# ChuckDanz/DCLIP

Measured on AMD Instinct MI355X. Metric: distill-step images/sec at ViT-B/32 bs=256, higher is better.
Workload: dtype f32

## Files before the change

### dclip_amd/_lib.py

```python
from __future__ import annotations

import ctypes as C
import os

_HERE = os.path.dirname(os.path.abspath(__file__))
LIB_PATH = os.environ.get("DCLIP_LIB_PATH") or os.path.join(_HERE, "libdclip_hip.so")

P = C.c_void_p
I = C.c_int
F = C.c_float
Z = C.c_size_t
L = C.c_int64

SIGNATURES = {
    "dclip_abi_version": (I, []),
    "dclip_last_error": (C.c_char_p, []),
    "dclip_last_launch": (C.c_char_p, []),
    "dclip_first_launch": (C.c_char_p, []),
    "dclip_gemm_f32_workspace": (Z, [I, I, I, I, I]),
    "dclip_gemm_f32_plan": (I, [I, I, I, I, I, C.POINTER(C.c_int)]),
    "dclip_gemm_f32": (I, [P, P, P, P, P, P, I, I, I, I, I, I, I, I, F, I, P, Z, P]),
    "dclip_colsum_f32_workspace": (Z, [I, I]),
    "dclip_colsum_f32": (I, [P, P, I, I, I, I, P, Z, P]),
    "dclip_layernorm_fwd": (I, [P, P, P, P, P, P, I, I, F, P]),
# ... 103 lines not shown
    "dclip_split_f32_f16x3_dev": (I, [P, P, I, I, I, I, P, I, P]),
    "dclip_layernorm_fwd_f16x3_dev": (I, [P, P, P, P, P, P, P, I, I, F, P, P]),
    "dclip_gemm_f16_scaled_dev": (I, [P, P, P, P, P, I, I, I, I, I, I, I, I, P, P]),
    "dclip_gemm_f16_scaled_split_dev": (I, [P, P, P, P, P, P, I, I, I, I, I, I, I, P, P, P]),
    "dclip_split16_record_bytes": (I, []),
    "dclip_split16_plan_floats": (I, []),
    "dclip_split16_tile_rows": (I, []),
    "dclip_split16_stats": (I, [P, I, I, P, P]),
    "dclip_split16_plan": (I, [P, P, I, I, P]),
    "dclip_split16_weights": (I, [P, I, I, P, P]),
    "dclip_split_f32_f16x3_rows": (I, [P, P, P, I, I, I, P]),
    "dclip_split16_weights_t": (I, [P, I, I, P, P, P]),
    "dclip_gemm_f16_scaled_rows_dev": (I, [P, P, P, P, I, I, I, I, I, I, I, P, P, P]),
    "dclip_split_f32_f16x3_rows_colstats_workspace": (Z, [I, I]),
    "dclip_split_f32_f16x3_rows_colstats": (I, [P, P, P, P, P, P, P, I, I, I, P, Z, P]),
    "dclip_split_f32_f16x3_rows_cols_stats": (I, [P, P, P, P, P, P, P, P, P, I, I, I, I, P]),
    "dclip_gemm_f16_scaled_rows_stats_plan": (I, [I, I, I]),
    "dclip_gemm_f16_scaled_rows_stats_dev": (I, [P, P, P, P, I, I, I, I, I, I, I, P, P, P, P, P]),
    "dclip_attention_bwd_stats_plan": (I, [I, I, I]),
    "dclip_attention_bwd_stats": (I, [P, P, P, P, P, P, P, I, I, I, I, P]),
    "dclip_layernorm_bwd_stats_plan": (I, [I, I]),
    "dclip_layernorm_bwd_stats": (I, [P, P, P, P, P, P, P, P, P, P, P, I, I, I, P, Z, P]),
    "dclip_gemm_f16x3_plan": (I, [I, I, I]),
    "dclip_gemm_f16x3_scaled": (I, [P, P, P, P, P, I, I, I, I, I, I, I, I, I, I, I, I, F, P]),
    "dclip_gemm_f16x3_scaled_split": (I, [P, P, P, P, I, I, I, I, I, I, I, I, I, I, I, F, F, P]),
    "dclip_gemm_f16x3_scaled_dev": (I, [P, P, P, P, P, I, I, I, I, I, I, I, I, I, I, I, I, P, P]),
    "dclip_gemm_f16x3_scaled_split_dev": (I, [P, P, P, P, P, P, I, I, I, I, I, I, I, I, I, I, I, P, P, P]),
    "dclip_gemm_f16x3_scaled_rows_dev": (I, [P, P, P, P, I, I, I, I, I, I, I, I, I, I, I, P, P, P]),
    "dclip_gemm_f16x3_scaled_rows_stats_plan": (I, [I, I, I]),
    "dclip_gemm_f16x3_scaled_rows_stats_dev": (I, [P, P, P, P, I, I, I, I, I, I, I, I, I, I, I, P, P, P, P, P]),
    "dclip_gemm_f16x3_wgrad_tokmajor_plan": (I, [I, I, I]),
    "dclip_gemm_f16x3_wgrad_tokmajor_workspace": (Z, [I, I, I]),
    "dclip_gemm_f16x3_wgrad_tokmajor": (I, [P, P, P, I, I, I, I, I, I, I, I, I, I, P, P, I, P, Z, P]),
    "dclip_gemm_f16_wgrad_tokmajor_seg3_plan": (I, [I, I, I]),
    "dclip_gemm_f16_wgrad_tokmajor_seg3": (I, [P, P, P, I, I, I, I, I, I, I, I, I, I, I, I, P, P, I, P, Z, P]),
    "dclip_gemm_f16_ex": (I, [P, P, P, P, P, P, I, I, I, I, I, I, I, I, P]),
    "dclip_gemm_f16_wgrad_tokmajor_plan": (I, [I, I, I]),
    "dclip_gemm_f16_wgrad_tokmajor": (I, [P, P, P, I, I, I, I, I, I, I, P, Z, P]),
    "dclip_gemm_f16_splitk_plan": (I, [I, I, I]),
    "dclip_gemm_f16_splitk_workspace": (Z, [I, I, I]),
    "dclip_gemm_f16_splitk": (I, [P, P, P, I, I, I, I, I, I, I, P, Z, P]),
    "dclip_cast_f32_f16_ieee": (I, [P, P, I, I, I, I, P]),
    "dclip_layernorm_fwd_f16_stats": (I, [P, P, P, P, P, P, I, I, F, P]),
    "dclip_layernorm_bwd_ex_f16": (I, [P, P, P, P, P, P, P, P, P, P, P, I, I, I, P, Z, P]),
    "dclip_transpose_to_f16": (I, [P, I, P, P, I, I, I, I, I, P]),
    "dclip_rowsum_f16": (I, [P, P, I, I, I, P]),
# ... 40 lines not shown
```

### dclip_amd/csrc/gemm_bf16.hip

```cpp
#include "common.h"
#include <stdlib.h>
#include <type_traits>

namespace {

typedef unsigned short u16x4 __attribute__((ext_vector_type(4)));
typedef unsigned int u32x4 __attribute__((ext_vector_type(4)));
typedef unsigned int u32x2 __attribute__((ext_vector_type(2)));

constexpr int BKH = 64;

struct GemmBf16Params {
  const __bf16* A;
  const __bf16* W;
  void* C;
  const float* bias;
  const float* residual;
  int M, N, K;
  int lda, ldw, ldc;
  int epilogue;
  int out_bf16;
  int tiles_m, tiles_n;
  unsigned short* aux;
  int k_per_split;
// ... 273 lines not shown
__device__ __forceinline__ void dma16(__amdgpu_buffer_rsrc_t rsrc, __bf16* lds_dst, int voff, int soff) {
  __builtin_amdgcn_raw_ptr_buffer_load_lds(rsrc, (__attribute__((address_space(3))) void*)lds_dst, 16, voff, soff, 0, 0);
}

template <class T, int BM>
int launch_reg(const GemmBf16Params& p, size_t lds, hipStream_t st) {
  if constexpr (std::is_same<T, F16T>::value) {
    if (p.row_alpha) {
      hipLaunchKernelGGL((gemm_bf16_kernel<T, BM, BM, true>), dim3(p.tiles_m * p.tiles_n), dim3(256), lds, st, p);
      return DCLIP_OK;
    }
  }
  hipLaunchKernelGGL((gemm_bf16_kernel<T, BM, BM>), dim3(p.tiles_m * p.tiles_n), dim3(256), lds, st, p);
  return DCLIP_OK;
}

#define PP_BARRIER()                      \
  do {                                    \
    __builtin_amdgcn_sched_barrier(0);    \
    __builtin_amdgcn_s_barrier();         \
    __builtin_amdgcn_sched_barrier(0);    \
  } while (0)

template <class T, int KIND, bool OUT16, bool DEV = false, bool ROWS = false, bool STATS = false>
__device__ __forceinline__ void pp_epilogue(const GemmBf16Params& p, const f32x4 (&acc)[8][4], float* ct, int m0, int n0,
                                            int tid, int wr, int wc, int quad, int l15) {
  constexpr int BN = 256;
  const int lc = (tid & 63) * 4, col = n0 + lc, lr0 = tid >> 6;
  const bool colok = col < p.N;
  const int colc = colok ? col : 0;
  f32x4 bias4 = {0.f, 0.f, 0.f, 0.f};
  if (p.epilogue & DCLIP_EPI_BIAS) bias4 = *reinterpret_cast<const f32x4*>(p.bias + colc);
  const float alpha_d = DEV ? *p.alpha_p : 0.f;
  static_assert(!STATS || ROWS, "the statistics form is the row-scaled one");
  unsigned smx[STATS ? 4 : 1];
  float ssm[STATS ? 4 : 1];
  if constexpr (STATS) {
#pragma unroll
    for (int e = 0; e < 4; ++e) smx[e] = 0u, ssm[e] = 0.f;
  }
#pragma unroll
  for (int hm = 0; hm < 2; ++hm) {
    const int rbase = m0 + hm * 128 + lr0;
    f32x4 side[KIND == 3 || (ROWS && KIND == 2) ? 16 : 1];
    u16x4 side16[KIND == 2 && !ROWS ? 16 : 1];
    if (ROWS && KIND == 2) {
#pragma unroll
      for (int q = 0; q < 16; ++q)
        side[q] = *reinterpret_cast<const f32x4*>(p.aux32 + (size_t)min(rbase + 8 * q, p.M - 1) * p.ldc + colc);
    }
    if (KIND == 3) {
#pragma unroll
      for (int q = 0; q < 16; ++q)
        side[q] = *reinterpret_cast<const f32x4*>(p.residual + (size_t)min(rbase + 8 * q, p.M - 1) * p.ldc + colc);
    }
    if (KIND == 2 && !ROWS) {
#pragma unroll
      for (int q = 0; q < 16; ++q)
        side16[q] = *reinterpret_cast<const u16x4*>(p.aux + (size_t)min(rbase + 8 * q, p.M - 1) * p.ldc + colc);
    }
    if (wr == hm) {
#pragma unroll
      for (int i = 0; i < 8; ++i)
#pragma unroll
        for (int j = 0; j < 4; ++j)
          *reinterpret_cast<f32x4*>(ct + (16 * i + l15) * BN + (((16 * wc + 4 * j + quad) ^ (l15 & 7)) << 2)) = acc[i][j];
    }
    asm volatile("s_waitcnt lgkmcnt(0)" ::: "memory");
    PP_BARRIER();
#pragma unroll
    for (int q = 0; q < 16; ++q) {
      const int row = rbase + 8 * q;
      f32x4 v = *reinterpret_cast<const f32x4*>(ct + (lr0 + 8 * q) * BN + (((tid & 63) ^ ((lr0 + 8 * q) & 7)) << 2));
      if (!ROWS) v = v * (DEV ? alpha_d : p.alpha) + bias4;
      const size_t off = (size_t)row * p.ldc + col;
      const bool ok = row < p.M && colok;
      if (ROWS) {
        if (KIND == 2) {
#pragma unroll
          for (int e = 0; e < 4; ++e) v[e] *= quick_gelu_grad_f(side[q][e]);
        }
        if (ok) *reinterpret_cast<f32x4*>(reinterpret_cast<float*>(p.C) + off) = v;
        if constexpr (STATS) if (ok) {
#pragma unroll
          for (int e = 0; e < 4; ++e) {
            const float ve = v[e];
            const unsigned u = __builtin_bit_cast(unsigned, ve) & 0x7fffffffu;
            smx[e] = smx[e] > u ? smx[e] : u;
            ssm[e] += ve;
          }
        }
        continue;
      }
      if (KIND == 1) {
        if (DEV && !OUT16 && p.h32 && ok) *reinterpret_cast<f32x4*>(p.h32 + (size_t)row * p.N + col) = v;
        if (p.aux) {
          u16x4 h = {T::bits(v[0]), T::bits(v[1]), T::bits(v[2]), T::bits(v[3])};
          if (ok) *reinterpret_cast<u16x4*>(p.aux + off) = h;
#pragma unroll
          for (int e = 0; e < 4; ++e) v[e] = T::to_f32(h[e]);
        }
#pragma unroll
        for (int e = 0; e < 4; ++e) v[e] = quick_gelu_f(v[e]);
      }
      if (KIND == 2) {
#pragma unroll
        for (int e = 0; e < 4; ++e) v[e] *= quick_gelu_grad_f(T::to_f32(side16[q][e]));
      }
      if (KIND == 3) v += side[q];
      if (!ok) continue;
      if ((KIND == 0 || KIND == 1) && !OUT16 && p.out_scale != 0.f) {
        if (DEV && p.g32) *reinterpret_cast<f32x4*>(p.g32 + (size_t)row * p.N + col) = v;
        store_split4(reinterpret_cast<unsigned short*>(p.C) + off, p.N, v, DEV ? *p.out_scale_p : p.out_scale);
        continue;
      }
      if (OUT16) {
        u16x4 o = {T::bits(v[0]), T::bits(v[1]), T::bits(v[2]), T::bits(v[3])};
        *reinterpret_cast<u16x4*>(reinterpret_cast<unsigned short*>(p.C) + off) = o;
      } else {
        *reinterpret_cast<f32x4*>(reinterpret_cast<float*>(p.C) + off) = v;
      }
    }
    if (hm == 0) {
      asm volatile("s_waitcnt lgkmcnt(0)" ::: "memory");
      PP_BARRIER();
      PP_STAMP(3);
    }
  }
  PP_STAMP(8);
  if constexpr (STATS) {
    asm volatile("s_waitcnt lgkmcnt(0)" ::: "memory");
    PP_BARRIER();
    unsigned* cu = reinterpret_cast<unsigned*>(ct);
    float* cs = ct + 8 * BN;
// ... 61 lines not shown
    if (row >= p.M || col >= p.N) continue;
    const size_t off = (size_t)row * p.ldc + col;
    const bool full = col + 8 <= p.N;
    typedef unsigned short u16x8 __attribute__((ext_vector_type(8)));
    u16x8 o = {lo[0], lo[1], lo[2], lo[3], hi[0], hi[1], hi[2], hi[3]};
    if (SAVE) {
      if (full) *reinterpret_cast<u16x8*>(p.aux + off) = o;
      else *reinterpret_cast<u16x4*>(p.aux + off) = lo;
#pragma unroll
      for (int e = 0; e < 8; ++e) o[e] = T::bits(quick_gelu_f(T::to_f32(o[e])));
    }
    unsigned short* c = reinterpret_cast<unsigned short*>(p.C) + off;
    if (full) *reinterpret_cast<u16x8*>(c) = o;
    else *reinterpret_cast<u16x4*>(c) = u16x4{o[0], o[1], o[2], o[3]};
  }
  PP_STAMP(8);
#ifdef DCLIP_GEMM_STAMPS
  asm volatile("s_waitcnt vmcnt(0)" ::: "memory");
#endif
  PP_STAMP(4);
  PP_STAMP_RT(6);
}

template <class T, bool TOK, bool DEV = false, bool ROWS = false, bool SEG = false, bool STATS = false, bool FUSED = false>
__global__ void __launch_bounds__(512) gemm_bf16_pp_kernel(GemmBf16Params p) {
  static_assert(!SEG || (TOK && !DEV && !ROWS), "the segmented form is token-major, split-K, fp32 slabs");
  static_assert(!FUSED || !SEG, "the fused form does all three products in one work item");
  constexpr int KT = FUSED ? BKH / 2 : BKH;
  static_assert(!STATS || (ROWS && !TOK), "the statistics form is the row-scaled dgrad");
  typedef typename T::x8 V8;
  constexpr int BM = 256, BN = 256, ROW = BKH;
  constexpr int BUF = (BM + BN) * ROW;
  __shared__ __attribute__((aligned(16))) unsigned char lds_raw[2 * BUF * 2];
  __bf16* lds = reinterpret_cast<__bf16*>(lds_raw);

  PP_STAMP(0);
  PP_STAMP_RT(5);
  PP_STAMP_V(7, (unsigned long long)__builtin_amdgcn_s_getreg((4) | (0 << 6) | (31 << 11)) |
                    ((unsigned long long)__builtin_amdgcn_s_getreg((20) | (0 << 6) | (3 << 11)) << 32));
  const int tid = threadIdx.x, lane = tid & 63;
  const int wave = __builtin_amdgcn_readfirstlane(tid >> 6);
  const int wr = wave >> 2, wc = wave & 3;
  const int l15 = lane & 15, quad = lane >> 4;

  constexpr int GROUP_M = 8;
  const int nwg = p.tiles_m * p.tiles_n;
  const int swz = xcd_remap16(blockIdx.x, nwg);
  const int per_group = GROUP_M * p.tiles_n;
  const int first_m = (swz / per_group) * GROUP_M;
  const int gsize = min(GROUP_M, p.tiles_m - first_m);
  const int tile_m = first_m + (swz % per_group) % gsize, tile_n = (swz % per_group) / gsize;
  const int m0 = tile_m * BM, n0 = tile_n * BN;
  int ksplit = blockIdx.y, a_col0 = 0, w_col0 = 0;
  if constexpr (SEG) {
    const int seg = (int)blockIdx.y / p.seg_splits;
    ksplit = (int)blockIdx.y - seg * p.seg_splits;
// ... 11 lines not shown
         w_bytes = TOK ? ((size_t)(p.K - kbeg - 1) * p.ldw + w_rows) * 2 : ((size_t)(w_rows - 1) * p.ldw + (p.K - kbeg)) * 2;
  if constexpr (FUSED) {
    a_bytes += (size_t)max(p.a_seg[0], p.a_seg[1]) * 2;
    w_bytes += (size_t)max(p.w_seg[0], p.w_seg[1]) * 2;
  }
  const __amdgpu_buffer_rsrc_t a_rsrc =
      __builtin_amdgcn_make_buffer_rsrc(const_cast<__bf16*>(a_org), 0, (int)min(a_bytes, (size_t)0x7fffffff), 0x00020000);
  const __amdgpu_buffer_rsrc_t w_rsrc =
      __builtin_amdgcn_make_buffer_rsrc(const_cast<__bf16*>(w_org), 0, (int)min(w_bytes, (size_t)0x7fffffff), 0x00020000);
  const int a_kstep = TOK ? KT * p.lda * 2 : KT * 2, w_kstep = TOK ? KT * p.ldw * 2 : KT * 2;
  int a_voff[2][2], w_voff[2][2];
#pragma unroll
  for (int h = 0; h < 2; ++h)
#pragma unroll
    for (int x = 0; x < 2; ++x) {
      if constexpr (FUSED) {
        if (TOK) {
          const int k = 4 * (wave + 8 * x) + (lane >> 4), tok = k & 31;
          const int lg = (lane & 15) ^ (((k & 3) << 2) | (((k >> 3) & 1) << 1));
          const int ma = 128 * (lg >> 3) + 64 * h + 8 * (lg & 7), nb = 64 * (lg >> 2) + 32 * h + 8 * (lg & 3);
          a_voff[h][x] = ma < a_rows ? (tok * p.lda + p.a_seg[x] + ma) * 2 : 0x7fffffff;
          w_voff[h][x] = nb < w_rows ? (tok * p.ldw + p.w_seg[x] + nb) * 2 : 0x7fffffff;
        } else {
          const int ra = 128 * x + 64 * h + 8 * wave + (lane >> 3), ga = (lane & 7) ^ ((ra >> 1) & 7);
          a_voff[h][x] = ra < a_rows ? (ra * p.lda + (ga < 4 ? p.a_seg[0] : p.a_seg[1]) + (ga & 3) * 8) * 2 : 0x7fffffff;
          const int rb = 64 * (2 * x + (wave >> 2)) + 32 * h + 8 * (wave & 3) + (lane >> 3), gb = (lane & 7) ^ ((rb >> 1) & 7);
          w_voff[h][x] = rb < w_rows ? (rb * p.ldw + (gb < 4 ? p.w_seg[0] : p.w_seg[1]) + (gb & 3) * 8) * 2 : 0x7fffffff;
        }
      } else if (TOK) {
        const int k = 4 * (wave + 8 * x) + (lane >> 4);
        const int lg = (lane & 15) ^ (((k & 3) << 2) | (((k >> 3) & 1) << 1));
        const int ma = 128 * (lg >> 3) + 64 * h + 8 * (lg & 7), nb = 64 * (lg >> 2) + 32 * h + 8 * (lg & 3);
        a_voff[h][x] = ma < a_rows ? (k * p.lda + ma) * 2 : 0x7fffffff;
        w_voff[h][x] = nb < w_rows ? (k * p.ldw + nb) * 2 : 0x7fffffff;
      } else {
        const int ra = 128 * x + 64 * h + 8 * wave + (lane >> 3), ga = (lane & 7) ^ ((ra >> 1) & 7);
        a_voff[h][x] = ra < a_rows ? (ra * p.lda + ga * 8) * 2 : 0x7fffffff;
        const int rb = 64 * (2 * x + (wave >> 2)) + 32 * h + 8 * (wave & 3) + (lane >> 3), gb = (lane & 7) ^ ((rb >> 1) & 7);
        w_voff[h][x] = rb < w_rows ? (rb * p.ldw + gb * 8) * 2 : 0x7fffffff;
      }
    }
  constexpr int HALF = 64 * 128;
#define PP_ISSUE_A(h, buf, kt)                                                                                          \
  do {                                                                                                                  \
    if (TOK) {                                                                                                          \
      dma16(a_rsrc, lds + (buf) * BUF + (h) * HALF + wave * 512, a_voff[h][0], (kt) * a_kstep);                         \
      dma16(a_rsrc, lds + (buf) * BUF + (h) * HALF + (wave + 8) * 512, a_voff[h][1], (kt) * a_kstep);                   \
    } else {                                                                                                            \
      dma16(a_rsrc, lds + (buf) * BUF + (64 * (h) + 8 * wave) * ROW, a_voff[h][0], (kt) * a_kstep);                     \
      dma16(a_rsrc, lds + (buf) * BUF + (128 + 64 * (h) + 8 * wave) * ROW, a_voff[h][1], (kt) * a_kstep);               \
    }                                                                                                                   \
  } while (0)
#define PP_ISSUE_B(h, buf, kt)                                                                                          \
  do {                                                                                                                  \
    if (TOK) {                                                                                                          \
      dma16(w_rsrc, lds + (buf) * BUF + (2 + (h)) * HALF + wave * 512, w_voff[h][0], (kt) * w_kstep);                   \
      dma16(w_rsrc, lds + (buf) * BUF + (2 + (h)) * HALF + (wave + 8) * 512, w_voff[h][1], (kt) * w_kstep);             \
    } else {                                                                                                            \
      dma16(w_rsrc, lds + (buf) * BUF + (BM + 64 * (wave >> 2) + 32 * (h) + 8 * (wave & 3)) * ROW, w_voff[h][0],        \
            (kt) * w_kstep);                                                                                            \
      dma16(w_rsrc, lds + (buf) * BUF + (BM + 128 + 64 * (wave >> 2) + 32 * (h) + 8 * (wave & 3)) * ROW, w_voff[h][1],  \
            (kt) * w_kstep);                                                                                            \
    }                                                                                                                   \
  } while (0)

  const int sw = l15 >> 1;
  const __bf16* pa0 = lds + (128 * wr + l15) * ROW + (((0 + quad) ^ sw) << 3);
  const __bf16* pa1 = lds + (128 * wr + l15) * ROW + (((4 + quad) ^ sw) << 3);
  const __bf16* pb0 = lds + (BM + 64 * wc + l15) * ROW + (((0 + quad) ^ sw) << 3);
  const __bf16* pb1 = lds + (BM + 64 * wc + l15) * ROW + (((4 + quad) ^ sw) << 3);
  const unsigned char* lds8 = lds_raw;
  const int tq = l15 >> 2, swzl = (tq << 2) | ((quad & 1) << 1);
  const int trow = (8 * quad + tq) * 256 + 8 * (l15 & 1);
  int ta[4], tb[2];
#pragma unroll
  for (int i = 0; i < 4; ++i) ta[i] = trow + (((8 * wr + 2 * i + ((l15 & 3) >> 1)) ^ swzl) << 4);
#pragma unroll
  for (int j = 0; j < 2; ++j) tb[j] = trow + (((4 * wc + 2 * j + ((l15 & 3) >> 1)) ^ swzl) << 4);
  auto tr8 = [&](int byte_off) {
    typedef short s16x4_t __attribute__((ext_vector_type(4)));
    typedef short s16x8_t __attribute__((ext_vector_type(8)));
    const s16x4_t lo = __builtin_amdgcn_ds_read_tr16_b64_v4i16((__attribute__((address_space(3))) s16x4_t*)(lds8 + byte_off));
    const s16x4_t hi = __builtin_amdgcn_ds_read_tr16_b64_v4i16((__attribute__((address_space(3))) s16x4_t*)(lds8 + byte_off + 1024));
    return __builtin_bit_cast(V8, s16x8_t{lo[0], lo[1], lo[2], lo[3], hi[0], hi[1], hi[2], hi[3]});
  };

  f32x4 acc[8][4];
#pragma unroll
  for (int i = 0; i < 8; ++i)
#pragma unroll
    for (int j = 0; j < 4; ++j) acc[i][j] = f32x4{0.f, 0.f, 0.f, 0.f};
  V8 fa[4][2], fb0[2][2], fb1[2][2];

#define PP_READ_A(qm, off)                                                                          \
  _Pragma("unroll") for (int i = 0; i < 4; ++i) {                                                   \
    if (TOK) {                                                                                      \
      fa[i][0] = tr8((off) * 2 + (qm) * (HALF * 2) + ta[i]);                                        \
      fa[i][1] = tr8((off) * 2 + (qm) * (HALF * 2) + ta[i] + 32 * 256);                             \
    } else {                                                                                        \
      fa[i][0] = *reinterpret_cast<const V8*>(pa0 + (off) + (64 * (qm) + 16 * i) * ROW);        \
      fa[i][1] = *reinterpret_cast<const V8*>(pa1 + (off) + (64 * (qm) + 16 * i) * ROW);        \
    }                                                                                               \
  }
#define PP_READ_B(fb, qn, off)                                                                      \
  _Pragma("unroll") for (int j = 0; j < 2; ++j) {                                                   \
    if (TOK) {                                                                                      \
      fb[j][0] = tr8((off) * 2 + (2 + (qn)) * (HALF * 2) + tb[j]);                                  \
      fb[j][1] = tr8((off) * 2 + (2 + (qn)) * (HALF * 2) + tb[j] + 32 * 256);                       \
    } else {                                                                                        \
      fb[j][0] = *reinterpret_cast<const V8*>(pb0 + (off) + (32 * (qn) + 16 * j) * ROW);        \
      fb[j][1] = *reinterpret_cast<const V8*>(pb1 + (off) + (32 * (qn) + 16 * j) * ROW);        \
    }                                                                                               \
  }
#define PP_MFMA(qm, qn, fb)                                                                                         \
  do {                                                                                                              \
    __builtin_amdgcn_s_setprio(1);                                                                                  \
    _Pragma("unroll") for (int s = 0; s < (FUSED ? 3 : 2); ++s)                                                     \
    _Pragma("unroll") for (int i = 0; i < 4; ++i)                                                                   \
    _Pragma("unroll") for (int j = 0; j < 2; ++j)                                                                   \
      acc[4 * (qm) + i][2 * (qn) + j] =                                                                             \
          T::mfma16(fb[j][FUSED ? s >> 1 : s], fa[i][FUSED ? s & 1 : s], acc[4 * (qm) + i][2 * (qn) + j]);          \
    __builtin_amdgcn_s_setprio(0);                                                                                  \
  } while (0)

  PP_ISSUE_A(0, 0, 0);
  PP_ISSUE_B(0, 0, 0);
  PP_ISSUE_B(1, 0, 0);
  PP_ISSUE_A(1, 0, 0);
  if (nk > 1) {
    PP_ISSUE_B(0, 1, 1);
    PP_ISSUE_A(0, 1, 1);
    PP_ISSUE_B(1, 1, 1);
    asm volatile("s_waitcnt vmcnt(6)" ::: "memory");
  } else {
    asm volatile("s_waitcnt vmcnt(0)" ::: "memory");
  }
  PP_BARRIER();
  PP_STAMP(1);
  if (wr == 1) PP_BARRIER();

  for (int kt = 0; kt < nk; ++kt) {
    const int cur = kt & 1, off = cur * BUF;
    const bool n1 = kt + 1 < nk, n2 = kt + 2 < nk;
    PP_READ_B(fb0, 0, off);
    __builtin_amdgcn_sched_barrier(0);
    PP_READ_A(0, off);
    __builtin_amdgcn_sched_barrier(0);
    if (n1) PP_ISSUE_A(1, cur ^ 1, kt + 1);
    if (!TOK) asm volatile("s_waitcnt lgkmcnt(8)" ::: "memory");
    PP_BARRIER();
    asm volatile("s_waitcnt lgkmcnt(0)" ::: "memory");
    __builtin_amdgcn_sched_barrier(0);
    PP_MFMA(0, 0, fb0);
    PP_BARRIER();
    PP_READ_B(fb1, 1, off);
    __builtin_amdgcn_sched_barrier(0);
    if (!TOK && n2) PP_ISSUE_B(0, cur, kt + 2);
    PP_BARRIER();
    asm volatile("s_waitcnt lgkmcnt(0)" ::: "memory");
    __builtin_amdgcn_sched_barrier(0);
    PP_MFMA(0, 1, fb1);
    PP_BARRIER();
    PP_READ_A(1, off);
    __builtin_amdgcn_sched_barrier(0);
    if (n2) PP_ISSUE_A(0, cur, kt + 2);
    PP_BARRIER();
    asm volatile("s_waitcnt lgkmcnt(0)" ::: "memory");
    __builtin_amdgcn_sched_barrier(0);
    PP_MFMA(1, 1, fb1);
    PP_BARRIER();
    if (n2) {
      if (TOK) PP_ISSUE_B(0, cur, kt + 2);
      PP_ISSUE_B(1, cur, kt + 2);
      asm volatile("s_waitcnt vmcnt(6)" ::: "memory");
    } else {
      asm volatile("s_waitcnt vmcnt(0)" ::: "memory");
    }
    PP_BARRIER();
    PP_MFMA(1, 0, fb0);
    PP_BARRIER();
  }
  if (wr == 0) PP_BARRIER();
  PP_STAMP(2);
#undef PP_ISSUE_A
#undef PP_ISSUE_B
#undef PP_READ_A
#undef PP_READ_B
#undef PP_MFMA

  const int kind = (p.epilogue & DCLIP_EPI_RESIDUAL) ? 3 : (p.epilogue & DCLIP_EPI_DGELU) ? 2 : (p.epilogue & DCLIP_EPI_GELU) ? 1 : 0;
  float* ct = reinterpret_cast<float*>(lds_raw);
  if (ROWS) {
    const float alpha_r = *p.alpha_p;
    float ra[8];
#pragma unroll
    for (int i = 0; i < 8; ++i) ra[i] = p.row_alpha[min(m0 + 128 * wr + 16 * i + l15, p.M - 1)];
#pragma unroll
    for (int i = 0; i < 8; ++i)
#pragma unroll
      for (int j = 0; j < 4; ++j) acc[i][j] = (acc[i][j] * alpha_r) * ra[i];
    if (kind == 2) pp_epilogue<T, 2, false, true, true, STATS>(p, acc, ct, m0, n0, tid, wr, wc, quad, l15);
    else pp_epilogue<T, 0, false, true, true, STATS>(p, acc, ct, m0, n0, tid, wr, wc, quad, l15);
    return;
  }
  if (!DEV && p.slab) {
    GemmBf16Params ps = p;
    ps.C = p.slab + (size_t)blockIdx.y * p.M * p.N;
    ps.ldc = p.N;
    ps.epilogue = 0;
    ps.alpha = 1.f;
    ps.out_scale = 0.f;
    pp_epilogue<T, 0, false, false>(ps, acc, ct, m0, n0, tid, wr, wc, quad, l15);
    return;
  }
  if (p.out_bf16) {
    unsigned short* ct16 = reinterpret_cast<unsigned short*>(lds_raw);
    if (kind == 0) pp_epilogue_b16<T, false, false, DEV>(p, acc, ct16, m0, n0, tid, wr, wc, quad, l15);
    else if (kind == 1 && p.aux) pp_epilogue_b16<T, true, true, DEV>(p, acc, ct16, m0, n0, tid, wr, wc, quad, l15);
    else if (kind == 1) pp_epilogue_b16<T, true, false, DEV>(p, acc, ct16, m0, n0, tid, wr, wc, quad, l15);
    else pp_epilogue<T, 2, true, DEV>(p, acc, ct, m0, n0, tid, wr, wc, quad, l15);
  } else {
    if (kind == 0) pp_epilogue<T, 0, false, DEV>(p, acc, ct, m0, n0, tid, wr, wc, quad, l15);
    else if (kind == 1) pp_epilogue<T, 1, false, DEV>(p, acc, ct, m0, n0, tid, wr, wc, quad, l15);
    else if (kind == 2) pp_epilogue<T, 2, false, DEV>(p, acc, ct, m0, n0, tid, wr, wc, quad, l15);
    else pp_epilogue<T, 3, false, DEV>(p, acc, ct, m0, n0, tid, wr, wc, quad, l15);
  }
}
#undef PP_BARRIER

#define PP_BARRIER()                      \
  do {                                    \
    __builtin_amdgcn_sched_barrier(0);    \
    __builtin_amdgcn_s_barrier();         \
    __builtin_amdgcn_sched_barrier(0);    \
  } while (0)

template <class T>
__global__ void __launch_bounds__(512) gemm_bf16_ppp_kernel(GemmBf16Params p) {
// ... 577 lines not shown
DCLIP_API int dclip_gemm_f16_scaled_rows_stats_dev(const void* A, const void* W, float* C, const float* aux32, int M, int N, int K,
                                                   int lda, int ldw, int ldc, int epilogue, const float* alpha, const float* row_alpha,
                                                   void* pmax, float* psum, void* stream) {
  DCLIP_REQUIRE(alpha && row_alpha && ((uintptr_t)alpha | (uintptr_t)row_alpha) % 4 == 0,
                "gemm_f16_scaled_rows_stats_dev: alpha / row_alpha must be device pointers");
  DCLIP_REQUIRE(pmax && psum && ((uintptr_t)pmax | (uintptr_t)psum) % 4 == 0, "gemm_f16_scaled_rows_stats_dev: pmax / psum");
  DCLIP_REQUIRE(epilogue == 0 || epilogue == DCLIP_EPI_DGELU, "gemm_f16_scaled_rows_stats_dev: the epilogue is none or DGELU");
  DCLIP_REQUIRE(!(epilogue & DCLIP_EPI_DGELU) || (aux32 && (uintptr_t)aux32 % 16 == 0),
                "gemm_f16_scaled_rows_stats_dev: DGELU needs a 16-byte aligned fp32 aux32");
  DCLIP_REQUIRE(dclip_gemm_f16_scaled_rows_stats_plan(M, N, K) > 0,
                "gemm_f16_scaled_rows_stats_dev: M=%d N=%d K=%d takes a register-staged kernel, which has no statistics form", M, N, K);
  DevScales dev{alpha, nullptr, nullptr, nullptr};
  dev.row_alpha = row_alpha;
  dev.aux32 = (epilogue & DCLIP_EPI_DGELU) ? aux32 : nullptr;
  dev.pmax = (unsigned*)pmax;
  dev.psum = psum;
  return gemm16<F16T>("gemm_f16_scaled_rows_dev.stats", A, W, C, nullptr, nullptr, nullptr, M, N, K, lda, ldw, ldc, epilogue, 0, stream,
                      1.f, 0.f, &dev);
}

namespace {
struct Segs { int a_hi, a_lo, w_hi, w_lo; };

int gemm16x3(const char* name, const void* A, const void* W, void* C, const float* bias, const float* residual, int M, int N, int K,
             int lda, int ldw, int ldc, Segs sg, int epilogue, int out_f16, void* stream, float alpha, float out_scale,
             const DevScales* dev) {
  DCLIP_REQUIRE(A && W && C, "%s: null operand", name);
  DCLIP_REQUIRE(M > 0 && N > 0 && K > 0 && K % 32 == 0, "%s: bad shape M=%d N=%d K=%d (K: the logical length, a multiple of 32)", name,
                M, N, K);
  DCLIP_REQUIRE(lda % 8 == 0 && ldw % 8 == 0 && lda > 0 && ldw > 0, "%s: lda/ldw must be multiples of 8", name);
  DCLIP_REQUIRE(sg.a_hi >= 0 && sg.a_lo >= 0 && sg.w_hi >= 0 && sg.w_lo >= 0 && (sg.a_hi | sg.a_lo | sg.w_hi | sg.w_lo) % 8 == 0,
                "%s: segment offsets must be non-negative multiples of 8", name);
  DCLIP_REQUIRE((long)sg.a_hi + K <= lda && (long)sg.a_lo + K <= lda && (long)sg.w_hi + K <= ldw && (long)sg.w_lo + K <= ldw,
                "%s: a segment (offset + K) must lie within the leading dimension", name);
  DCLIP_REQUIRE(N % 4 == 0 && ldc % 4 == 0 && ldc >= N, "%s: N / ldc must be multiples of 4", name);
  DCLIP_REQUIRE(((uintptr_t)A | (uintptr_t)W | (uintptr_t)C) % 16 == 0, "%s: operands must be 16-byte aligned", name);
  DCLIP_REQUIRE(!(epilogue & ~(DCLIP_EPI_BIAS | DCLIP_EPI_GELU | DCLIP_EPI_DGELU | DCLIP_EPI_RESIDUAL)),
                "%s: unsupported epilogue bits", name);
  DCLIP_REQUIRE(out_scale == 0.f || (!out_f16 && !(epilogue & (DCLIP_EPI_RESIDUAL | DCLIP_EPI_DGELU)) && (long)ldc >= 3L * N),
                "%s: a split output takes BIAS | GELU only and ldc >= 3 N", name);
  DCLIP_REQUIRE(!(epilogue & DCLIP_EPI_DGELU) || (dev && dev->aux32 && !(epilogue & DCLIP_EPI_GELU)), "%s: DGELU needs aux32", name);
  DCLIP_REQUIRE(!(epilogue & DCLIP_EPI_BIAS) || bias, "%s: BIAS without bias", name);
  DCLIP_REQUIRE(!(epilogue & DCLIP_EPI_RESIDUAL) || (residual && !out_f16), "%s: RESIDUAL needs an fp32 output", name);
  DCLIP_REQUIRE(256L * lda * 2 < 0x7fffffffL && 256L * ldw * 2 < 0x7fffffffL, "%s: leading dimension too large", name);
  GemmBf16Params p{(const __bf16*)A, (const __bf16*)W, C, bias, residual, M, N, K, lda, ldw, ldc, epilogue, out_f16, cdiv(M, 256),
                   cdiv(N, 256), nullptr, 0, nullptr, alpha, out_scale};
  set_dev(p, dev);
  p.a_seg[0] = sg.a_hi, p.a_seg[1] = sg.a_lo, p.w_seg[0] = sg.w_hi, p.w_seg[1] = sg.w_lo;
  const dim3 grid(p.tiles_m * p.tiles_n), block(512);
  hipStream_t st = (hipStream_t)stream;
  if (p.row_alpha && p.pmax)
    hipLaunchKernelGGL((gemm_bf16_pp_kernel<F16T, false, true, true, false, true, true>), grid, block, 0, st, p);
  else if (p.row_alpha)
    hipLaunchKernelGGL((gemm_bf16_pp_kernel<F16T, false, true, true, false, false, true>), grid, block, 0, st, p);
  else if (p.alpha_p)
    hipLaunchKernelGGL((gemm_bf16_pp_kernel<F16T, false, true, false, false, false, true>), grid, block, 0, st, p);
  else
    hipLaunchKernelGGL((gemm_bf16_pp_kernel<F16T, false, false, false, false, false, true>), grid, block, 0, st, p);
  DCLIP_CHECK_LAUNCH_V(name, ".pp3");
  return DCLIP_OK;
}
}

DCLIP_API int dclip_gemm_f16x3_plan(int M, int N, int K) {
  if (M <= 0 || N <= 0 || K <= 0 || K % 32 != 0 || !takes_pp(M, N, 3 * K)) return 0;
  const int tiles_min = getenv("DCLIP_F16X3_MIN") ? atoi(getenv("DCLIP_F16X3_MIN")) : 128;
  return (long)cdiv(M, 256) * cdiv(N, 256) >= tiles_min ? 1 : 0;
}

DCLIP_API int dclip_gemm_f16x3_scaled(const void* A, const void* W, void* C, const float* bias, const float* residual, int M, int N,
                                      int K, int lda, int ldw, int ldc, int a_hi, int a_lo, int w_hi, int w_lo, int epilogue,
                                      int out_f16, float alpha, void* stream) {
  DCLIP_REQUIRE(!(epilogue & DCLIP_EPI_DGELU), "gemm_f16x3_scaled: DGELU is a training epilogue");
  DCLIP_REQUIRE(alpha == alpha && alpha - alpha == 0.f, "gemm_f16x3_scaled: alpha must be finite");
  return gemm16x3("gemm_f16x3_scaled", A, W, C, bias, residual, M, N, K, lda, ldw, ldc, Segs{a_hi, a_lo, w_hi, w_lo}, epilogue, out_f16,
                  stream, alpha, 0.f, nullptr);
}

DCLIP_API int dclip_gemm_f16x3_scaled_split(const void* A, const void* W, void* C, const float* bias, int M, int N, int K, int lda,
                                            int ldw, int ldc, int a_hi, int a_lo, int w_hi, int w_lo, int epilogue, float alpha,
                                            float out_scale, void* stream) {
  DCLIP_REQUIRE(alpha == alpha && alpha - alpha == 0.f, "gemm_f16x3_scaled_split: alpha must be finite");
  DCLIP_REQUIRE(out_scale > 0.f && out_scale - out_scale == 0.f && (__builtin_bit_cast(unsigned int, out_scale) & 0x007fffffu) == 0,
                "gemm_f16x3_scaled_split: out_scale must be a power of two");
  DCLIP_REQUIRE(ldc % 8 == 0, "gemm_f16x3_scaled_split: ldc must be a multiple of 8");
  return gemm16x3("gemm_f16x3_scaled_split", A, W, C, bias, nullptr, M, N, K, lda, ldw, ldc, Segs{a_hi, a_lo, w_hi, w_lo}, epilogue, 0,
                  stream, alpha, out_scale, nullptr);
}

DCLIP_API int dclip_gemm_f16x3_scaled_dev(const void* A, const void* W, void* C, const float* bias, const float* residual, int M,
// ... 385 lines not shown
```

### dclip_amd/ops.py

```python
from __future__ import annotations

from typing import Optional

import torch

from . import _lib

A_KMAJOR, B_KMAJOR = 1, 2
EPI_BIAS, EPI_GELU, EPI_DGELU, EPI_RESIDUAL, EPI_ACCUM, EPI_A_ROWSUM = 1, 2, 4, 8, 16, 32
LAYOUT_NT = A_KMAJOR | B_KMAJOR
LAYOUT_NN = A_KMAJOR
LAYOUT_TN = 0


def _stream():
    return torch.cuda.current_stream().cuda_stream


def _f32(t: torch.Tensor, name: str) -> torch.Tensor:
    if not (t.is_cuda and t.dtype == torch.float32 and t.is_contiguous()):
        raise ValueError(f"{name}: expected a contiguous float32 CUDA tensor, got {t.dtype} {t.device} "
                         f"contiguous={t.is_contiguous()}")
    return t

# ... 1359 lines not shown
    a_seg = (0, M, 0) if a_seg is None else tuple(int(v) for v in a_seg)
    w_seg = (0, 0, N) if w_seg is None else tuple(int(v) for v in w_seg)
    if splits is None:
        splits = lib.dclip_gemm_f16_wgrad_tokmajor_seg3_plan(M, N, tokens)
        if splits == 0:
            return None
    if _f32(col_alpha, "col_alpha").numel() != M:
        raise ValueError("gemm_f16_wgrad_tokmajor_seg3: col_alpha size")
    out = _out_f32(out, (M, N), dy.device, "gemm_f16_wgrad_tokmajor_seg3")
    nbytes = lib.dclip_gemm_f16_splitk_workspace(M, N, 3 * splits)
    ws = _ws.get(nbytes, dy.device)
    _lib.check(lib.dclip_gemm_f16_wgrad_tokmajor_seg3(dy.data_ptr(), x.data_ptr(), out.data_ptr(), M, N, tokens, dy.shape[1], x.shape[1],
                                                      N, a_seg[0], a_seg[1], a_seg[2], w_seg[0], w_seg[1], w_seg[2],
                                                      col_alpha.data_ptr(), act_scale_ptr, splits, _ptr(ws), nbytes, _stream()),
               "gemm_f16_wgrad_tokmajor_seg3")
    return out



def gemm_f16x3_plan(M: int, N: int, K: int) -> int:
    return int(_lib.load().dclip_gemm_f16x3_plan(M, N, K))


def _x3_k(a: torch.Tensor, w: torch.Tensor, name: str):
    _f16(a, "a"), _f16(w, "w")
    M, lda = a.shape
    N, ldw = w.shape
    if min(lda, ldw) % 3:
        raise ValueError(f"{name}: a / w are [rows, 3 K] splits")
    K = min(lda, ldw) // 3
    return M, N, K, lda, ldw


def gemm_f16x3(a: torch.Tensor, w: torch.Tensor, *, bias: Optional[torch.Tensor] = None, residual: Optional[torch.Tensor] = None,
               gelu: bool = False, out_f16: bool = False, alpha: float = 1.0, split_out_scale: Optional[float] = None,
               segs=None) -> torch.Tensor:
    lib = _lib.load()
    M, N, K, lda, ldw = _x3_k(a, w, "gemm_f16x3")
    sg = (0, K, 0, 2 * K) if segs is None else tuple(int(v) for v in segs)
    epi = 0
    if bias is not None:
        epi |= EPI_BIAS
        if _f32(bias, "bias").numel() != N:
            raise ValueError("gemm_f16x3: bias size")
    if gelu:
        epi |= EPI_GELU
# ... 588 lines not shown
```

### include/dclip_hip.h

```cpp
#ifndef DCLIP_HIP_H
#define DCLIP_HIP_H

#include <stddef.h>
#include <stdint.h>

#ifdef __cplusplus
extern "C" {
#endif

#define DCLIP_ABI_VERSION 1

enum {
  DCLIP_OK = 0,
  DCLIP_EINVAL = -1,
  DCLIP_EWORKSPACE = -2,
  DCLIP_ELAUNCH = -3
};

int dclip_abi_version(void);
const char* dclip_last_error(void);
const char* dclip_last_launch(void);
const char* dclip_first_launch(void);

#define DCLIP_A_KMAJOR 1
// ... 226 lines not shown
size_t dclip_split_f32_f16x3_rows_colstats_workspace(int rows, int cols);
int dclip_split_f32_f16x3_rows_colstats(const float* x, void* y, float* row_alpha, void* yc, int* col_exp, float* col_alpha, float* db,
                                        int rows, int cols, int ldx, void* workspace, size_t workspace_bytes, void* stream);
int dclip_gemm_f16_wgrad_tokmajor_seg3_plan(int M, int N, int tokens);
int dclip_gemm_f16_wgrad_tokmajor_seg3(const void* dY, const void* X, float* C, int M, int N, int tokens, int lddy, int ldx, int ldc,
                                       int a_seg0, int a_seg1, int a_seg2, int w_seg0, int w_seg1, int w_seg2, const float* col_alpha,
                                       const float* act_scale, int splits, void* workspace, size_t workspace_bytes, void* stream);

int dclip_split_f32_f16x3_rows_cols_stats(const float* x, void* y, float* row_alpha, void* yc, int* col_exp, float* col_alpha, float* db,
                                          const void* pmax, const float* psum, int P, int rows, int cols, int ldx, void* stream);
int dclip_gemm_f16_scaled_rows_stats_plan(int M, int N, int K);
int dclip_gemm_f16_scaled_rows_stats_dev(const void* A, const void* W, float* C, const float* aux32, int M, int N, int K, int lda,
                                         int ldw, int ldc, int epilogue, const float* alpha, const float* row_alpha, void* pmax,
                                         float* psum, void* stream);
int dclip_attention_bwd_stats_plan(int B, int S, int H);
int dclip_attention_bwd_stats(const float* qkv, const float* out, const float* dout, const float* lse, float* dqkv, void* pmax,
                              float* psum, int B, int S, int H, int causal, void* stream);
int dclip_layernorm_bwd_stats_plan(int rows, int D);
int dclip_layernorm_bwd_stats(const float* dy, const float* x, const float* gamma, const float* mean, const float* rstd,
                              const float* dresidual, float* dx, float* dgamma, float* dbeta, void* pmax, float* psum, int rows, int D,
                              int accumulate_param_grads, void* workspace, size_t workspace_bytes, void* stream);

int dclip_gemm_f16x3_plan(int M, int N, int K);
int dclip_gemm_f16x3_scaled(const void* A, const void* W, void* C, const float* bias, const float* residual, int M, int N, int K,
                            int lda, int ldw, int ldc, int a_hi, int a_lo, int w_hi, int w_lo, int epilogue, int out_f16, float alpha,
                            void* stream);
int dclip_gemm_f16x3_scaled_split(const void* A, const void* W, void* C, const float* bias, int M, int N, int K, int lda, int ldw,
                                  int ldc, int a_hi, int a_lo, int w_hi, int w_lo, int epilogue, float alpha, float out_scale,
                                  void* stream);
int dclip_gemm_f16x3_scaled_dev(const void* A, const void* W, void* C, const float* bias, const float* residual, int M, int N, int K,
                                int lda, int ldw, int ldc, int a_hi, int a_lo, int w_hi, int w_lo, int epilogue, int out_f16,
                                const float* alpha, void* stream);
int dclip_gemm_f16x3_scaled_split_dev(const void* A, const void* W, void* C, const float* bias, float* h32, float* g32, int M, int N,
                                      int K, int lda, int ldw, int ldc, int a_hi, int a_lo, int w_hi, int w_lo, int epilogue,
                                      const float* alpha, const float* out_scale, void* stream);
int dclip_gemm_f16x3_scaled_rows_dev(const void* A, const void* W, float* C, const float* aux32, int M, int N, int K, int lda, int ldw,
                                     int ldc, int a_hi, int a_lo, int w_hi, int w_lo, int epilogue, const float* alpha,
                                     const float* row_alpha, void* stream);
int dclip_gemm_f16x3_scaled_rows_stats_plan(int M, int N, int K);
int dclip_gemm_f16x3_scaled_rows_stats_dev(const void* A, const void* W, float* C, const float* aux32, int M, int N, int K, int lda,
                                           int ldw, int ldc, int a_hi, int a_lo, int w_hi, int w_lo, int epilogue, const float* alpha,
                                           const float* row_alpha, void* pmax, float* psum, void* stream);
int dclip_gemm_f16x3_wgrad_tokmajor_plan(int M, int N, int tokens);
size_t dclip_gemm_f16x3_wgrad_tokmajor_workspace(int M, int N, int splits);
int dclip_gemm_f16x3_wgrad_tokmajor(const void* dY, const void* X, float* C, int M, int N, int tokens, int lddy, int ldx, int ldc,
                                    int dy_hi, int dy_lo, int x_hi, int x_lo, const float* col_alpha, const float* act_scale,
// ... 41 lines not shown
```

Measured before the change: 7856.

## Add a 192-row tile variant of the fused f16x3 GEMM to cut wave quantization

```diff
diff --git a/dclip_amd/_lib.py b/dclip_amd/_lib.py
--- a/dclip_amd/_lib.py
+++ b/dclip_amd/_lib.py
@@ -149,6 +149,7 @@
     "dclip_layernorm_bwd_stats_plan": (I, [I, I]),
     "dclip_layernorm_bwd_stats": (I, [P, P, P, P, P, P, P, P, P, P, P, I, I, I, P, Z, P]),
     "dclip_gemm_f16x3_plan": (I, [I, I, I]),
+    "dclip_gemm_f16x3_tile_rows": (I, [I, I, I, I, I]),
     "dclip_gemm_f16x3_scaled": (I, [P, P, P, P, P, I, I, I, I, I, I, I, I, I, I, I, I, F, P]),
     "dclip_gemm_f16x3_scaled_split": (I, [P, P, P, P, I, I, I, I, I, I, I, I, I, I, I, F, F, P]),
     "dclip_gemm_f16x3_scaled_dev": (I, [P, P, P, P, P, I, I, I, I, I, I, I, I, I, I, I, I, P, P]),
diff --git a/dclip_amd/csrc/gemm_bf16.hip b/dclip_amd/csrc/gemm_bf16.hip
--- a/dclip_amd/csrc/gemm_bf16.hip
+++ b/dclip_amd/csrc/gemm_bf16.hip
@@ -319,10 +319,11 @@
     __builtin_amdgcn_sched_barrier(0);    \
   } while (0)
 
-template <class T, int KIND, bool OUT16, bool DEV = false, bool ROWS = false, bool STATS = false>
-__device__ __forceinline__ void pp_epilogue(const GemmBf16Params& p, const f32x4 (&acc)[8][4], float* ct, int m0, int n0,
+template <class T, int KIND, bool OUT16, bool DEV = false, bool ROWS = false, bool STATS = false, int BM = 256>
+__device__ __forceinline__ void pp_epilogue(const GemmBf16Params& p, const f32x4 (&acc)[BM / 32][4], float* ct, int m0, int n0,
                                             int tid, int wr, int wc, int quad, int l15) {
-  constexpr int BN = 256;
+  constexpr int BN = 256, WM = BM / 2, NQ = WM / 8;
+  static_assert(BM == 256 || (BM == 192 && !OUT16 && !STATS), "the 192-row tile has fp32 outputs and no statistics form");
   const int lc = (tid & 63) * 4, col = n0 + lc, lr0 = tid >> 6;
   const bool colok = col < p.N;
   const int colc = colok ? col : 0;
@@ -338,27 +339,27 @@
   }
 #pragma unroll
   for (int hm = 0; hm < 2; ++hm) {
-    const int rbase = m0 + hm * 128 + lr0;
-    f32x4 side[KIND == 3 || (ROWS && KIND == 2) ? 16 : 1];
-    u16x4 side16[KIND == 2 && !ROWS ? 16 : 1];
+    const int rbase = m0 + hm * WM + lr0;
+    f32x4 side[KIND == 3 || (ROWS && KIND == 2) ? NQ : 1];
+    u16x4 side16[KIND == 2 && !ROWS ? NQ : 1];
     if (ROWS && KIND == 2) {
 #pragma unroll
-      for (int q = 0; q < 16; ++q)
+      for (int q = 0; q < NQ; ++q)
         side[q] = *reinterpret_cast<const f32x4*>(p.aux32 + (size_t)min(rbase + 8 * q, p.M - 1) * p.ldc + colc);
     }
     if (KIND == 3) {
 #pragma unroll
-      for (int q = 0; q < 16; ++q)
+      for (int q = 0; q < NQ; ++q)
         side[q] = *reinterpret_cast<const f32x4*>(p.residual + (size_t)min(rbase + 8 * q, p.M - 1) * p.ldc + colc);
     }
     if (KIND == 2 && !ROWS) {
 #pragma unroll
-      for (int q = 0; q < 16; ++q)
+      for (int q = 0; q < NQ; ++q)
         side16[q] = *reinterpret_cast<const u16x4*>(p.aux + (size_t)min(rbase + 8 * q, p.M - 1) * p.ldc + colc);
     }
     if (wr == hm) {
 #pragma unroll
-      for (int i = 0; i < 8; ++i)
+      for (int i = 0; i < BM / 32; ++i)
 #pragma unroll
         for (int j = 0; j < 4; ++j)
           *reinterpret_cast<f32x4*>(ct + (16 * i + l15) * BN + (((16 * wc + 4 * j + quad) ^ (l15 & 7)) << 2)) = acc[i][j];
@@ -366,7 +367,7 @@
     asm volatile("s_waitcnt lgkmcnt(0)" ::: "memory");
     PP_BARRIER();
 #pragma unroll
-    for (int q = 0; q < 16; ++q) {
+    for (int q = 0; q < NQ; ++q) {
       const int row = rbase + 8 * q;
       f32x4 v = *reinterpret_cast<const f32x4*>(ct + (lr0 + 8 * q) * BN + (((tid & 63) ^ ((lr0 + 8 * q) & 7)) << 2));
       if (!ROWS) v = v * (DEV ? alpha_d : p.alpha) + bias4;
@@ -406,7 +407,7 @@
       }
       if (KIND == 3) v += side[q];
       if (!ok) continue;
-      if ((KIND == 0 || KIND == 1) && !OUT16 && p.out_scale != 0.f) {
+      if (BM == 256 && (KIND == 0 || KIND == 1) && !OUT16 && p.out_scale != 0.f) {
         if (DEV && p.g32) *reinterpret_cast<f32x4*>(p.g32 + (size_t)row * p.N + col) = v;
         store_split4(reinterpret_cast<unsigned short*>(p.C) + off, p.N, v, DEV ? *p.out_scale_p : p.out_scale);
         continue;
@@ -514,16 +515,20 @@
   PP_STAMP_RT(6);
 }
 
-template <class T, bool TOK, bool DEV = false, bool ROWS = false, bool SEG = false, bool STATS = false, bool FUSED = false>
+template <class T, bool TOK, bool DEV = false, bool ROWS = false, bool SEG = false, bool STATS = false, bool FUSED = false,
+          int BM = 256>
 __global__ void __launch_bounds__(512) gemm_bf16_pp_kernel(GemmBf16Params p) {
   static_assert(!SEG || (TOK && !DEV && !ROWS), "the segmented form is token-major, split-K, fp32 slabs");
   static_assert(!FUSED || !SEG, "the fused form does all three products in one work item");
   constexpr int KT = FUSED ? BKH / 2 : BKH;
   static_assert(!STATS || (ROWS && !TOK), "the statistics form is the row-scaled dgrad");
+  static_assert(BM == 256 || (BM == 192 && FUSED && !TOK && !SEG && !STATS), "the 192-row tile is K-major, fused, no statistics");
   typedef typename T::x8 V8;
-  constexpr int BM = 256, BN = 256, ROW = BKH;
+  constexpr int BN = 256, ROW = BKH;
+  constexpr int WM = BM / 2, QM = WM / 2, IB = QM / 16;
   constexpr int BUF = (BM + BN) * ROW;
-  __shared__ __attribute__((aligned(16))) unsigned char lds_raw[2 * BUF * 2];
+  constexpr int DUMP = BM == 256 ? 0 : 8 * 1024;
+  __shared__ __attribute__((aligned(16))) unsigned char lds_raw[2 * BUF * 2 + DUMP];
   __bf16* lds = reinterpret_cast<__bf16*>(lds_raw);
 
   PP_STAMP(0);
@@ -581,7 +586,9 @@
           a_voff[h][x] = ma < a_rows ? (tok * p.lda + p.a_seg[x] + ma) * 2 : 0x7fffffff;
           w_voff[h][x] = nb < w_rows ? (tok * p.ldw + p.w_seg[x] + nb) * 2 : 0x7fffffff;
         } else {
-          const int ra = 128 * x + 64 * h + 8 * wave + (lane >> 3), ga = (lane & 7) ^ ((ra >> 1) & 7);
+          const int qa = wave + 8 * x;
+          const int ra = (BM == 256 ? 128 * x + 64 * h + 8 * wave : qa < 12 ? WM * (qa / 6) + QM * h + 8 * (qa % 6) : BM) + (lane >> 3);
+          const int ga = (lane & 7) ^ ((ra >> 1) & 7);
           a_voff[h][x] = ra < a_rows ? (ra * p.lda + (ga < 4 ? p.a_seg[0] : p.a_seg[1]) + (ga & 3) * 8) * 2 : 0x7fffffff;
           const int rb = 64 * (2 * x + (wave >> 2)) + 32 * h + 8 * (wave & 3) + (lane >> 3), gb = (lane & 7) ^ ((rb >> 1) & 7);
           w_voff[h][x] = rb < w_rows ? (rb * p.ldw + (gb < 4 ? p.w_seg[0] : p.w_seg[1]) + (gb & 3) * 8) * 2 : 0x7fffffff;
@@ -600,11 +607,17 @@
       }
     }
   constexpr int HALF = 64 * 128;
+  const int a192_e0 = (WM * (wave / 6) + 8 * (wave % 6)) * ROW;
+  const bool a192_in = wave < 4;
+  const int a192_e1 = a192_in ? (WM + 8 * (wave + 2)) * ROW : 2 * BUF + wave * 512;
 #define PP_ISSUE_A(h, buf, kt)                                                                                          \
   do {                                                                                                                  \
     if (TOK) {                                                                                                          \
       dma16(a_rsrc, lds + (buf) * BUF + (h) * HALF + wave * 512, a_voff[h][0], (kt) * a_kstep);                         \
       dma16(a_rsrc, lds + (buf) * BUF + (h) * HALF + (wave + 8) * 512, a_voff[h][1], (kt) * a_kstep);                   \
+    } else if (BM == 192) {                                                                                             \
+      dma16(a_rsrc, lds + (buf) * BUF + QM * (h) * ROW + a192_e0, a_voff[h][0], (kt) * a_kstep);                        \
+      dma16(a_rsrc, lds + (a192_in ? (buf) * BUF + QM * (h) * ROW : 0) + a192_e1, a_voff[h][1], (kt) * a_kstep);        \
     } else {                                                                                                            \
       dma16(a_rsrc, lds + (buf) * BUF + (64 * (h) + 8 * wave) * ROW, a_voff[h][0], (kt) * a_kstep);                     \
       dma16(a_rsrc, lds + (buf) * BUF + (128 + 64 * (h) + 8 * wave) * ROW, a_voff[h][1], (kt) * a_kstep);               \
@@ -624,8 +637,8 @@
   } while (0)
 
   const int sw = l15 >> 1;
-  const __bf16* pa0 = lds + (128 * wr + l15) * ROW + (((0 + quad) ^ sw) << 3);
-  const __bf16* pa1 = lds + (128 * wr + l15) * ROW + (((4 + quad) ^ sw) << 3);
+  const __bf16* pa0 = lds + (WM * wr + l15) * ROW + (((0 + quad) ^ sw) << 3);
+  const __bf16* pa1 = lds + (WM * wr + l15) * ROW + (((4 + quad) ^ sw) << 3);
   const __bf16* pb0 = lds + (BM + 64 * wc + l15) * ROW + (((0 + quad) ^ sw) << 3);
   const __bf16* pb1 = lds + (BM + 64 * wc + l15) * ROW + (((4 + quad) ^ sw) << 3);
   const unsigned char* lds8 = lds_raw;
@@ -644,21 +657,21 @@
     return __builtin_bit_cast(V8, s16x8_t{lo[0], lo[1], lo[2], lo[3], hi[0], hi[1], hi[2], hi[3]});
   };
 
-  f32x4 acc[8][4];
-#pragma unroll
-  for (int i = 0; i < 8; ++i)
+  f32x4 acc[2 * IB][4];
+#pragma unroll
+  for (int i = 0; i < 2 * IB; ++i)
 #pragma unroll
     for (int j = 0; j < 4; ++j) acc[i][j] = f32x4{0.f, 0.f, 0.f, 0.f};
-  V8 fa[4][2], fb0[2][2], fb1[2][2];
+  V8 fa[IB][2], fb0[2][2], fb1[2][2];
 
 #define PP_READ_A(qm, off)                                                                          \
-  _Pragma("unroll") for (int i = 0; i < 4; ++i) {                                                   \
+  _Pragma("unroll") for (int i = 0; i < IB; ++i) {                                                  \
     if (TOK) {                                                                                      \
       fa[i][0] = tr8((off) * 2 + (qm) * (HALF * 2) + ta[i]);                                        \
       fa[i][1] = tr8((off) * 2 + (qm) * (HALF * 2) + ta[i] + 32 * 256);                             \
     } else {                                                                                        \
-      fa[i][0] = *reinterpret_cast<const V8*>(pa0 + (off) + (64 * (qm) + 16 * i) * ROW);        \
-      fa[i][1] = *reinterpret_cast<const V8*>(pa1 + (off) + (64 * (qm) + 16 * i) * ROW);        \
+      fa[i][0] = *reinterpret_cast<const V8*>(pa0 + (off) + (QM * (qm) + 16 * i) * ROW);        \
+      fa[i][1] = *reinterpret_cast<const V8*>(pa1 + (off) + (QM * (qm) + 16 * i) * ROW);        \
     }                                                                                               \
   }
 #define PP_READ_B(fb, qn, off)                                                                      \
@@ -675,10 +688,10 @@
   do {                                                                                                              \
     __builtin_amdgcn_s_setprio(1);                                                                                  \
     _Pragma("unroll") for (int s = 0; s < (FUSED ? 3 : 2); ++s)                                                     \
-    _Pragma("unroll") for (int i = 0; i < 4; ++i)                                                                   \
+    _Pragma("unroll") for (int i = 0; i < IB; ++i)                                                                  \
     _Pragma("unroll") for (int j = 0; j < 2; ++j)                                                                   \
-      acc[4 * (qm) + i][2 * (qn) + j] =                                                                             \
-          T::mfma16(fb[j][FUSED ? s >> 1 : s], fa[i][FUSED ? s & 1 : s], acc[4 * (qm) + i][2 * (qn) + j]);          \
+      acc[IB * (qm) + i][2 * (qn) + j] =                                                                            \
+          T::mfma16(fb[j][FUSED ? s >> 1 : s], fa[i][FUSED ? s & 1 : s], acc[IB * (qm) + i][2 * (qn) + j]);         \
     __builtin_amdgcn_s_setprio(0);                                                                                  \
   } while (0)
 
@@ -706,7 +719,8 @@
     PP_READ_A(0, off);
     __builtin_amdgcn_sched_barrier(0);
     if (n1) PP_ISSUE_A(1, cur ^ 1, kt + 1);
-    if (!TOK) asm volatile("s_waitcnt lgkmcnt(8)" ::: "memory");
+    if (!TOK && BM == 256) asm volatile("s_waitcnt lgkmcnt(8)" ::: "memory");
+    if (!TOK && BM == 192) asm volatile("s_waitcnt lgkmcnt(6)" ::: "memory");
     PP_BARRIER();
     asm volatile("s_waitcnt lgkmcnt(0)" ::: "memory");
     __builtin_amdgcn_sched_barrier(0);
@@ -751,15 +765,15 @@
   float* ct = reinterpret_cast<float*>(lds_raw);
   if (ROWS) {
     const float alpha_r = *p.alpha_p;
-    float ra[8];
-#pragma unroll
-    for (int i = 0; i < 8; ++i) ra[i] = p.row_alpha[min(m0 + 128 * wr + 16 * i + l15, p.M - 1)];
-#pragma unroll
-    for (int i = 0; i < 8; ++i)
+    float ra[2 * IB];
+#pragma unroll
+    for (int i = 0; i < 2 * IB; ++i) ra[i] = p.row_alpha[min(m0 + WM * wr + 16 * i + l15, p.M - 1)];
+#pragma unroll
+    for (int i = 0; i < 2 * IB; ++i)
 #pragma unroll
       for (int j = 0; j < 4; ++j) acc[i][j] = (acc[i][j] * alpha_r) * ra[i];
-    if (kind == 2) pp_epilogue<T, 2, false, true, true, STATS>(p, acc, ct, m0, n0, tid, wr, wc, quad, l15);
-    else pp_epilogue<T, 0, false, true, true, STATS>(p, acc, ct, m0, n0, tid, wr, wc, quad, l15);
+    if (kind == 2) pp_epilogue<T, 2, false, true, true, STATS, BM>(p, acc, ct, m0, n0, tid, wr, wc, quad, l15);
+    else pp_epilogue<T, 0, false, true, true, STATS, BM>(p, acc, ct, m0, n0, tid, wr, wc, quad, l15);
     return;
   }
   if (!DEV && p.slab) {
@@ -769,10 +783,15 @@
     ps.epilogue = 0;
     ps.alpha = 1.f;
     ps.out_scale = 0.f;
-    pp_epilogue<T, 0, false, false>(ps, acc, ct, m0, n0, tid, wr, wc, quad, l15);
+    pp_epilogue<T, 0, false, false, false, false, BM>(ps, acc, ct, m0, n0, tid, wr, wc, quad, l15);
     return;
   }
-  if (p.out_bf16) {
+  if constexpr (BM == 192) {
+    if (kind == 0) pp_epilogue<T, 0, false, DEV, false, false, BM>(p, acc, ct, m0, n0, tid, wr, wc, quad, l15);
+    else if (kind == 1) pp_epilogue<T, 1, false, DEV, false, false, BM>(p, acc, ct, m0, n0, tid, wr, wc, quad, l15);
+    else if (kind == 2) pp_epilogue<T, 2, false, DEV, false, false, BM>(p, acc, ct, m0, n0, tid, wr, wc, quad, l15);
+    else pp_epilogue<T, 3, false, DEV, false, false, BM>(p, acc, ct, m0, n0, tid, wr, wc, quad, l15);
+  } else if (p.out_bf16) {
     unsigned short* ct16 = reinterpret_cast<unsigned short*>(lds_raw);
     if (kind == 0) pp_epilogue_b16<T, false, false, DEV>(p, acc, ct16, m0, n0, tid, wr, wc, quad, l15);
     else if (kind == 1 && p.aux) pp_epilogue_b16<T, true, true, DEV>(p, acc, ct16, m0, n0, tid, wr, wc, quad, l15);
@@ -1396,6 +1415,18 @@
 namespace {
 struct Segs { int a_hi, a_lo, w_hi, w_lo; };
 
+constexpr int kBm192CostPct = 91;
+int f16x3_tile_rows(int M, int N, bool has192) {
+  const int mode = getenv("DCLIP_F16X3_BM192") ? atoi(getenv("DCLIP_F16X3_BM192")) : 1;
+  if (!has192 || mode <= 0) return 256;
+  if (mode >= 2) return 192;
+  const int tiles_min = getenv("DCLIP_F16X3_BM192_MIN") ? atoi(getenv("DCLIP_F16X3_BM192_MIN")) : 128;
+  const long t256 = (long)cdiv(M, 256) * cdiv(N, 256), t192 = (long)cdiv(M, 192) * cdiv(N, 256);
+  if (t256 < tiles_min) return 256;
+  const long r256 = (t256 + 255) / 256, r192 = (t192 + 255) / 256;
+  return r192 * kBm192CostPct < r256 * 100 ? 192 : 256;
+}
+
 int gemm16x3(const char* name, const void* A, const void* W, void* C, const float* bias, const float* residual, int M, int N, int K,
              int lda, int ldw, int ldc, Segs sg, int epilogue, int out_f16, void* stream, float alpha, float out_scale,
              const DevScales* dev) {
@@ -1417,12 +1448,24 @@
   DCLIP_REQUIRE(!(epilogue & DCLIP_EPI_BIAS) || bias, "%s: BIAS without bias", name);
   DCLIP_REQUIRE(!(epilogue & DCLIP_EPI_RESIDUAL) || (residual && !out_f16), "%s: RESIDUAL needs an fp32 output", name);
   DCLIP_REQUIRE(256L * lda * 2 < 0x7fffffffL && 256L * ldw * 2 < 0x7fffffffL, "%s: leading dimension too large", name);
-  GemmBf16Params p{(const __bf16*)A, (const __bf16*)W, C, bias, residual, M, N, K, lda, ldw, ldc, epilogue, out_f16, cdiv(M, 256),
+  const bool has192 = !out_f16 && out_scale == 0.f && !(dev && dev->pmax);
+  const int bm = f16x3_tile_rows(M, N, has192);
+  GemmBf16Params p{(const __bf16*)A, (const __bf16*)W, C, bias, residual, M, N, K, lda, ldw, ldc, epilogue, out_f16, cdiv(M, bm),
                    cdiv(N, 256), nullptr, 0, nullptr, alpha, out_scale};
   set_dev(p, dev);
   p.a_seg[0] = sg.a_hi, p.a_seg[1] = sg.a_lo, p.w_seg[0] = sg.w_hi, p.w_seg[1] = sg.w_lo;
   const dim3 grid(p.tiles_m * p.tiles_n), block(512);
   hipStream_t st = (hipStream_t)stream;
+  if (bm == 192) {
+    if (p.row_alpha)
+      hipLaunchKernelGGL((gemm_bf16_pp_kernel<F16T, false, true, true, false, false, true, 192>), grid, block, 0, st, p);
+    else if (p.alpha_p)
+      hipLaunchKernelGGL((gemm_bf16_pp_kernel<F16T, false, true, false, false, false, true, 192>), grid, block, 0, st, p);
+    else
+      hipLaunchKernelGGL((gemm_bf16_pp_kernel<F16T, false, false, false, false, false, true, 192>), grid, block, 0, st, p);
+    DCLIP_CHECK_LAUNCH_V(name, ".pp3_192");
+    return DCLIP_OK;
+  }
   if (p.row_alpha && p.pmax)
     hipLaunchKernelGGL((gemm_bf16_pp_kernel<F16T, false, true, true, false, true, true>), grid, block, 0, st, p);
   else if (p.row_alpha)
@@ -1440,6 +1483,12 @@
   if (M <= 0 || N <= 0 || K <= 0 || K % 32 != 0 || !takes_pp(M, N, 3 * K)) return 0;
   const int tiles_min = getenv("DCLIP_F16X3_MIN") ? atoi(getenv("DCLIP_F16X3_MIN")) : 128;
   return (long)cdiv(M, 256) * cdiv(N, 256) >= tiles_min ? 1 : 0;
+}
+
+DCLIP_API int dclip_gemm_f16x3_tile_rows(int M, int N, int K, int rows_form, int stats_form) {
+  (void)K, (void)rows_form;
+  if (M <= 0 || N <= 0) return 256;
+  return f16x3_tile_rows(M, N, !stats_form);
 }
 
 DCLIP_API int dclip_gemm_f16x3_scaled(const void* A, const void* W, void* C, const float* bias, const float* residual, int M, int N,
diff --git a/dclip_amd/ops.py b/dclip_amd/ops.py
--- a/dclip_amd/ops.py
+++ b/dclip_amd/ops.py
@@ -1405,6 +1405,10 @@
     return int(_lib.load().dclip_gemm_f16x3_plan(M, N, K))
 
 
+def gemm_f16x3_tile_rows(M: int, N: int, K: int, rows_form: bool = False, stats_form: bool = False) -> int:
+    return int(_lib.load().dclip_gemm_f16x3_tile_rows(M, N, K, int(rows_form), int(stats_form)))
+
+
 def _x3_k(a: torch.Tensor, w: torch.Tensor, name: str):
     _f16(a, "a"), _f16(w, "w")
     M, lda = a.shape
diff --git a/include/dclip_hip.h b/include/dclip_hip.h
--- a/include/dclip_hip.h
+++ b/include/dclip_hip.h
@@ -272,6 +272,7 @@
                               int accumulate_param_grads, void* workspace, size_t workspace_bytes, void* stream);
 
 int dclip_gemm_f16x3_plan(int M, int N, int K);
+int dclip_gemm_f16x3_tile_rows(int M, int N, int K, int rows_form, int stats_form);
 int dclip_gemm_f16x3_scaled(const void* A, const void* W, void* C, const float* bias, const float* residual, int M, int N, int K,
                             int lda, int ldw, int ldc, int a_hi, int a_lo, int w_hi, int w_lo, int epilogue, int out_f16, float alpha,
                             void* stream);
```

Result: faster. 7955 (median of 6 runs) (+1.3%).
